# PhyloStar/CyBayes

Measured on NVIDIA B200. Metric: tree log-likelihood evals/sec, higher is better.
Workload: dtype f64

## Files before the change

### cybayes_b200/csrc/cybayes_b200.cu

```cuda
#include <cuda_runtime.h>
#include <dlfcn.h>
#include <limits.h>
#include <stdarg.h>
#include <stdio.h>
#include <stdlib.h>
#include <string.h>

#include <time.h>

#include <algorithm>
#include <exception>
#include <new>
#include <string>
#include <vector>

#include "cb_types.cuh"
#include "kernels_dmma.cuh"
#include "kernels_dmma_rc.cuh"
#include "kernels_general.cuh"
#include "kernels_pmat.cuh"
#include "kernels_s2.cuh"
#include "kernels_s2t.cuh"

using namespace cb;
// ... 36 lines not shown
  } catch (...) {
    return fail("internal error: unknown exception");
  }
}

struct NcclId { char internal[128]; };
typedef struct ncclComm* ncclComm_t;
struct NcclApi {
  void* lib = nullptr;
  int (*GetUniqueId)(NcclId*) = nullptr;
  int (*CommInitRank)(ncclComm_t*, int, NcclId, int) = nullptr;
  int (*AllReduce)(const void*, void*, size_t, int, int, ncclComm_t, cudaStream_t) = nullptr;
  int (*AllGather)(const void*, void*, size_t, int, ncclComm_t, cudaStream_t) = nullptr;
  int (*CommDestroy)(ncclComm_t) = nullptr;
  const char* (*GetErrorString)(int) = nullptr;
};
static NcclApi g_nccl;
static int load_nccl() {
  if (g_nccl.lib) return 0;
  const char* names[] = {"libnccl.so.2", "libnccl.so"};
  for (const char* n : names) {
    g_nccl.lib = dlopen(n, RTLD_NOW | RTLD_GLOBAL);
    if (g_nccl.lib) break;
  }
  REQUIRE(g_nccl.lib, "cannot dlopen libnccl.so.2: %s", dlerror());
  g_nccl.GetUniqueId = (int (*)(NcclId*))dlsym(g_nccl.lib, "ncclGetUniqueId");
  g_nccl.CommInitRank = (int (*)(ncclComm_t*, int, NcclId, int))dlsym(g_nccl.lib, "ncclCommInitRank");
  g_nccl.AllReduce = (int (*)(const void*, void*, size_t, int, int, ncclComm_t, cudaStream_t))dlsym(g_nccl.lib, "ncclAllReduce");
  g_nccl.AllGather = (int (*)(const void*, void*, size_t, int, ncclComm_t, cudaStream_t))dlsym(g_nccl.lib, "ncclAllGather");
  g_nccl.CommDestroy = (int (*)(ncclComm_t))dlsym(g_nccl.lib, "ncclCommDestroy");
  g_nccl.GetErrorString = (const char* (*)(int))dlsym(g_nccl.lib, "ncclGetErrorString");
  REQUIRE(g_nccl.GetUniqueId && g_nccl.CommInitRank && g_nccl.AllReduce && g_nccl.CommDestroy,
          "libnccl is missing expected symbols");
  return 0;
}
enum { NCCL_DOUBLE = 8, NCCL_SUM = 0, NCCL_INT8 = 0 };

constexpr int DMMA_RC_MIN_STATES = 9;
constexpr int64_t DMMA_RC_MIN_SITES = 1024;
constexpr int64_t S2_TILED_MIN_SITES = 64 * 2 * 148 * 4;

struct Buffer {
  double* data = nullptr;
  int32_t* scale = nullptr;
  int refs = 0;
};
struct Snapshot {
  std::vector<int32_t> buf_of_node;
  std::vector<int32_t> cherry_of_node;
  int refs = 0;
};
struct CherryRec {
  int32_t tip[2] = {0, 0};
  int refs = 0;
};

struct PlanChild {
  int32_t kind;
  int32_t ref;
  int32_t edge;
};
struct PlanOp {
  int32_t node;
  PlanChild ch[2];
  int32_t out_buf;
  int32_t pf_buf;
  uint8_t is_root, keep, stream, spill, pushed;
  uint8_t make_rec;
  uint8_t synthetic;
};
struct PlanLaunch { int r_begin, r_end, max_ops, n_bufs; };
struct EvalPlan {
  int flags = 0, n_lists = 0, split_env = 0;
  std::vector<int32_t> key_offsets, key_nodes, key_children;
  std::vector<PlanOp> ops;
  std::vector<RangeDesc> ranges;
  std::vector<PlanLaunch> launches;
  int64_t bytes_written = 0, bytes_read = 0;
  int n_stored = 0, n_buffer_reads = 0, n_stack = 0, n_spills = 0, n_cherries = 0, n_small_recs = 0;
  uint64_t stamp = 0;
};
constexpr int PLAN_FLAG_MASK = CB_EVAL_WANT_SNAPSHOT | CB_EVAL_STORE_ROOT | CB_EVAL_FORCE_LEVELS | CB_EVAL_FORCE_WALK | CB_EVAL_NO_FOLD;
constexpr int PLAN_CACHE_SIZE = 6;

struct cb_ctx {
  int device = 0;
  cudaStream_t stream = nullptr;
  cudaEvent_t ev0 = nullptr, ev1 = nullptr, ev_stage = nullptr, ev_mark[2] = {nullptr, nullptr};
  int sm_count = 148;
  int n_taxa = 0, n_states = 0, n_cats = 0, code_bytes = 1, n_amb = 0;
  int64_t n_sites = 0, P = 0;
  bool family_s2 = false;
  bool use_dmma = false;
  bool dmma_rc = false;
  int rc_stagger = 1;
  double* d_staged = nullptr;
  size_t staged_bytes = 0;
  bool s2_tiled = false;
  int s2t_slots = 3;
  int s2t_minb = 3;
  int s2t_v = 2;
  bool s2t_bulk = false;
  bool s2t_prefetch = true;
  bool s2t_small_recs = true;
  S2TImage* d_images = nullptr;
  int s2_vec = 1;
  int s2_minb = 3;
  bool s2_stream_stores = true;
  void* d_codes = nullptr;
  double* d_weights = nullptr;
  double* d_amb = nullptr;
  double* d_pi = nullptr;
  double* d_pmats = nullptr;
  int pmat_cap = 0;
  std::vector<Buffer> buffers;
  std::vector<int> free_buffers;
  size_t buffer_bytes = 0;
  std::vector<Snapshot> snaps;
  std::vector<int> free_snaps;
  std::vector<CherryRec> recs;
  std::vector<int> free_recs;
  double* d_pmats_lib = nullptr;
  int lib_cap = 0;
  unsigned char* h_stage = nullptr;
  unsigned char* d_stage = nullptr;
  size_t stage_cap = 0;
  int images_cap = 0;
  cudaEvent_t ev_scratch = nullptr;
  bool timing = true;
  bool results_mapped = false;
  double* d_block_sums = nullptr;
  unsigned* d_tickets = nullptr;
  double* d_results = nullptr;
  double* h_results = nullptr;
  double* d_root_dot = nullptr;
  int32_t* d_root_exp = nullptr;
  int out_cap = 0, max_blocks = 0;
  int last_n_out = 0;
  void* d_scratch = nullptr;
  void* h_scratch = nullptr;
  size_t scratch_cap = 0;
  void* d_flush = nullptr;
  size_t flush_bytes = 0;
  ncclComm_t comm = nullptr;
  int n_ranks = 1, rank = 0;
  bool fused_allreduce = false;
  Mail* d_mailbox = nullptr;
  Mail** d_peer_mailbox = nullptr;
  std::vector<void*> peer_opened;
  int32_t* d_comm_error = nullptr;
  unsigned long long epoch = 0;
  std::vector<EvalPlan> plans;
  EvalPlan scratch_plan;
  uint64_t plan_clock = 0, plan_builds = 0;
  bool no_plan_cache = false;
  std::vector<int> work_new_bufs, work_new_nodes, work_cherry_nodes;
  cudaEvent_t ev_main0 = nullptr, ev_main1 = nullptr;
// ... 23 lines not shown
  dev_account(c->device, (int64_t)bytes);
  return 0;
}
static void dev_free(cb_ctx* c, void* p, size_t bytes) {
  if (p) {
    cudaFree(p);
    c->dev_bytes -= (int64_t)bytes;
    dev_account(c->device, -(int64_t)bytes);
  }
}

extern "C" const char* cb_last_error(void) { return g_err.c_str(); }
extern "C" int cb_version(void) { return 100; }
extern "C" int cb_device_count(int* out) {
  REQUIRE(out, "null argument");
  CU(cudaGetDeviceCount(out));
  return 0;
}

static int create_impl(int device, cb_ctx** out);
extern "C" int cb_create(int device, cb_ctx** out) {
  return guarded([&] { return create_impl(device, out); });
}
static int create_impl(int device, cb_ctx** out) {
  REQUIRE(out, "null argument");
  int n = 0;
  cudaError_t e = cudaGetDeviceCount(&n);
  if (e != cudaSuccess || n == 0)
    return fail("no CUDA device available (%s); cybayes_b200 has no CPU fallback", cudaGetErrorString(e));
  REQUIRE(device >= 0 && device < n, "device %d out of range (have %d)", device, n);
  CU(cudaSetDevice(device));
  cb_ctx* c = new cb_ctx();
  c->device = device;
  CU(cudaStreamCreateWithFlags(&c->stream, cudaStreamNonBlocking));
  CU(cudaEventCreate(&c->ev0));
  CU(cudaEventCreate(&c->ev1));
  CU(cudaEventCreateWithFlags(&c->ev_stage, cudaEventDisableTiming));
  CU(cudaEventCreate(&c->ev_mark[0]));
  CU(cudaEventCreate(&c->ev_mark[1]));
  CU(cudaEventCreateWithFlags(&c->ev_scratch, cudaEventDisableTiming));
  CU(cudaEventCreate(&c->ev_main0));
  CU(cudaEventCreate(&c->ev_main1));
  cudaDeviceProp prop;
  CU(cudaGetDeviceProperties(&prop, device));
  c->sm_count = prop.multiProcessorCount;
  if (const char* v = getenv("CYBAYES_S2_V")) c->s2_vec = (atoi(v) == 2) ? 2 : 1;
  if (const char* v = getenv("CYBAYES_S2_MINB")) c->s2_minb = (atoi(v) == 4) ? 4 : 3;
  if (getenv("CYBAYES_S2_NO_CS")) c->s2_stream_stores = false;
  if (const char* v = getenv("CYBAYES_S2T_MINB")) c->s2t_minb = std::max(2, std::min(4, atoi(v)));
  if (const char* v = getenv("CYBAYES_S2T_V")) c->s2t_v = atoi(v) == 2 ? 2 : 1;
  if (c->s2t_minb == 4) c->s2t_v = 1;
  if (getenv("CYBAYES_S2T_BULK")) c->s2t_bulk = atoi(getenv("CYBAYES_S2T_BULK")) != 0;
  if (getenv("CYBAYES_S2T_PREFETCH")) c->s2t_prefetch = atoi(getenv("CYBAYES_S2T_PREFETCH")) != 0;
  if (getenv("CYBAYES_S2T_SMALL_RECS")) c->s2t_small_recs = atoi(getenv("CYBAYES_S2T_SMALL_RECS")) != 0;
  c->s2t_slots = c->s2t_minb == 4 ? 2 : c->s2t_minb == 3 ? 3 : 4;
  if (const char* v = getenv("CYBAYES_S2T_SLOTS")) c->s2t_slots = std::max(0, std::min(8, atoi(v)));
  if (getenv("CYBAYES_NO_PLAN_CACHE")) c->no_plan_cache = true;
  if (const char* v = getenv("CYBAYES_MAX_DEVICE_BYTES")) c->max_dev_bytes = atoll(v);
#define CB_S2T_ATTR(CC, MB, VV) CU(cudaFuncSetAttribute(prune_s2t_kernel<CC, MB, VV>, cudaFuncAttributeMaxDynamicSharedMemorySize, 226 * 1024))
  CB_S2T_ATTR(4, 2, 1); CB_S2T_ATTR(4, 3, 1); CB_S2T_ATTR(1, 2, 1); CB_S2T_ATTR(1, 3, 1);
  CB_S2T_ATTR(4, 2, 2); CB_S2T_ATTR(1, 2, 2); CB_S2T_ATTR(4, 3, 2); CB_S2T_ATTR(1, 3, 2); CB_S2T_ATTR(4, 4, 1); CB_S2T_ATTR(1, 4, 1);
#undef CB_S2T_ATTR
  CU(cudaFuncSetAttribute(prune_general_kernel, cudaFuncAttributeMaxDynamicSharedMemorySize, 227 * 1024));
#define CB_DMMA_ATTR(SS) CU(cudaFuncSetAttribute(prune_dmma_kernel<SS>, cudaFuncAttributeMaxDynamicSharedMemorySize, 227 * 1024))
  CB_DMMA_ATTR(0); CB_DMMA_ATTR(32); CB_DMMA_ATTR(40); CB_DMMA_ATTR(47); CB_DMMA_ATTR(48); CB_DMMA_ATTR(56); CB_DMMA_ATTR(64);
#undef CB_DMMA_ATTR
#define CB_RC_ATTR(SS)                                                                                                          \
  CU(cudaFuncSetAttribute(prune_dmma_rc_kernel<SS, true>, cudaFuncAttributeMaxDynamicSharedMemorySize, (int)RcCfg<SS>::SMEM)); \
  CU(cudaFuncSetAttribute(prune_dmma_rc_kernel<SS, false>, cudaFuncAttributeMaxDynamicSharedMemorySize, (int)RcCfg<SS>::SMEM))
  CB_RC_ATTR(16); CB_RC_ATTR(24); CB_RC_ATTR(32); CB_RC_ATTR(40); CB_RC_ATTR(48); CB_RC_ATTR(56); CB_RC_ATTR(64);
#undef CB_RC_ATTR
  if (const char* v = getenv("CYBAYES_RC_STAGGER")) c->rc_stagger = atoi(v) != 0;
  *out = c;
  return 0;
}

static void free_alignment(cb_ctx* c) {
  c->plans.clear();
  if (c->d_images) dev_free(c, c->d_images, (size_t)c->images_cap * sizeof(S2TImage));
  c->d_images = nullptr;
  c->images_cap = 0;
  for (auto& b : c->buffers) dev_free(c, b.data, c->buffer_bytes);
  c->buffers.clear();
  c->free_buffers.clear();
  c->snaps.clear();
  c->free_snaps.clear();
  c->recs.clear();
  c->free_recs.clear();
  if (c->d_pmats_lib) dev_free(c, c->d_pmats_lib, (size_t)c->lib_cap * 2 * c->n_cats * c->n_states * c->n_states * 8);
  c->d_pmats_lib = nullptr;
  c->lib_cap = 0;
  if (c->d_codes) dev_free(c, c->d_codes, (size_t)c->n_taxa * c->P * c->code_bytes);
  if (c->d_weights) dev_free(c, c->d_weights, (size_t)c->P * 8);
  if (c->d_amb) dev_free(c, c->d_amb, (size_t)std::max(1, c->n_amb) * c->n_states * 8);
  if (c->d_pi) dev_free(c, c->d_pi, (size_t)c->n_states * 8);
  if (c->d_pmats) dev_free(c, c->d_pmats, (size_t)c->pmat_cap * c->n_states * c->n_states * 8);
  if (c->d_staged) dev_free(c, c->d_staged, c->staged_bytes);
  c->d_staged = nullptr;
  c->staged_bytes = 0;
  c->d_codes = nullptr;
  c->d_weights = c->d_amb = c->d_pi = c->d_pmats = nullptr;
  c->pmat_cap = 0;
  if (c->d_block_sums) dev_free(c, c->d_block_sums, (size_t)c->out_cap * c->max_blocks * 8);
  if (c->d_tickets) dev_free(c, c->d_tickets, (size_t)c->out_cap * 4);
  if (c->d_results) dev_free(c, c->d_results, (size_t)c->out_cap * 8);
  if (c->d_root_dot) dev_free(c, c->d_root_dot, (size_t)c->out_cap * c->n_cats * c->P * 8);
  if (c->d_root_exp) dev_free(c, c->d_root_exp, (size_t)c->out_cap * c->n_cats * c->P * 4);
// ... 243 lines not shown
  if (check_slots(c, count, slots)) return 1;
  REQUIRE(d, "null argument");
  REQUIRE(model >= CB_MODEL_JC && model <= CB_MODEL_GTR_EIG, "unknown model %d", model);
  REQUIRE(model == CB_MODEL_JC || pi, "pi required");
  REQUIRE(model != CB_MODEL_GTR_EIG || gtr, "GTR eigensystem required");
  REQUIRE(model != CB_MODEL_F81_BINARY || c->n_states == 2, "binary F81 needs 2 states");
  if (count == 0) return 0;
  CU(cudaSetDevice(c->device));
  const int S = c->n_states;
  const size_t n_gtr = (model == CB_MODEL_GTR_EIG) ? (size_t)S + 2 * (size_t)S * S : 0;
  const size_t doubles = (size_t)S + n_gtr + 2 * (size_t)count;
  const size_t bytes = doubles * 8 + (size_t)count * 4;
  if (ensure_scratch(c, bytes)) return 1;
  CU(cudaEventSynchronize(c->ev_scratch));
  double* h = (double*)c->h_scratch;
  if (pi) memcpy(h, pi, (size_t)S * 8); else memset(h, 0, (size_t)S * 8);
  if (n_gtr) memcpy(h + S, gtr, n_gtr * 8);
  memcpy(h + S + n_gtr, d, (size_t)count * 8);
  if (x) memcpy(h + S + n_gtr + count, x, (size_t)count * 8);
  memcpy(h + doubles, slots, (size_t)count * 4);
  CU(cudaMemcpyAsync(c->d_scratch, c->h_scratch, bytes, cudaMemcpyHostToDevice, c->stream));
  CU(cudaEventRecord(c->ev_scratch, c->stream));
  c->h2d += (int64_t)bytes;
  const double* dd = (const double*)c->d_scratch;
  const int threads = (S * S >= 256) ? 256 : ((S * S + 31) / 32 * 32);
  pmat_build_kernel<<<count, threads, (size_t)S * 8, c->stream>>>(
      model, S, dd, beta, n_gtr ? dd + S : nullptr, count, (const int32_t*)(dd + doubles), dd + S + n_gtr,
      x ? dd + S + n_gtr + count : nullptr, c->d_pmats);
  CU(cudaGetLastError());
  c->launches += 1;
  return 0;
}

static int buffer_acquire(cb_ctx* c, int* out) {
  if (!c->free_buffers.empty()) {
    *out = c->free_buffers.back();
    c->free_buffers.pop_back();
  } else {
    Buffer b;
    void* p = nullptr;
    if (dev_alloc(c, &p, c->buffer_bytes)) return 1;
    b.data = (double*)p;
    b.scale = (int32_t*)(b.data + (size_t)c->n_cats * c->n_states * c->P);
    c->buffers.push_back(b);
    *out = (int)c->buffers.size() - 1;
  }
  c->buffers[*out].refs = 1;
  return 0;
}
static void buffer_release(cb_ctx* c, int b) {
  if (b < 0) return;
  if (--c->buffers[b].refs == 0) c->free_buffers.push_back(b);
}
static int rec_acquire(cb_ctx* c, int tip0, int tip1, int* out) {
  if (!c->free_recs.empty()) {
    *out = c->free_recs.back();
    c->free_recs.pop_back();
  } else {
    c->recs.emplace_back();
    *out = (int)c->recs.size() - 1;
  }
  c->recs[*out].tip[0] = tip0;
  c->recs[*out].tip[1] = tip1;
  c->recs[*out].refs = 1;
  return 0;
}
static void rec_release(cb_ctx* c, int r) {
  if (r < 0) return;
  if (--c->recs[r].refs == 0) c->free_recs.push_back(r);
}
static int ensure_lib_pool(cb_ctx* c) {
  const int need = (int)c->recs.size();
  if (need <= c->lib_cap) return 0;
  const int cap = std::max(need, std::max(1024, c->lib_cap * 2));
  const size_t per = (size_t)2 * c->n_cats * c->n_states * c->n_states * 8;
  double* nd = nullptr;
  if (dev_alloc(c, (void**)&nd, (size_t)cap * per)) return 1;
  if (c->d_pmats_lib) {
    CU(cudaMemcpyAsync(nd, c->d_pmats_lib, (size_t)c->lib_cap * per, cudaMemcpyDeviceToDevice, c->stream));
    CU(cudaStreamSynchronize(c->stream));
    dev_free(c, c->d_pmats_lib, (size_t)c->lib_cap * per);
  }
  c->d_pmats_lib = nd;
  c->lib_cap = cap;
  return 0;
}
static bool snapshot_valid(cb_ctx* c, int s) {
  return s >= 0 && s < (int)c->snaps.size() && c->snaps[s].refs > 0;
}
extern "C" int cb_snapshot_retain(cb_ctx* c, int s) {
  REQUIRE(c && snapshot_valid(c, s), "invalid snapshot %d", s);
  c->snaps[s].refs++;
  return 0;
}
extern "C" int cb_snapshot_release(cb_ctx* c, int s) {
  REQUIRE(c && snapshot_valid(c, s), "invalid snapshot %d", s);
  if (--c->snaps[s].refs == 0) {
    for (int32_t b : c->snaps[s].buf_of_node) buffer_release(c, b);
    for (int32_t r : c->snaps[s].cherry_of_node) rec_release(c, r);
    c->snaps[s].buf_of_node.clear();
    c->snaps[s].cherry_of_node.clear();
    c->free_snaps.push_back(s);
  }
  return 0;
}

static int snapshot_read_impl(cb_ctx* c, int s, int node, double* out, int32_t* scale_out);
extern "C" int cb_snapshot_read(cb_ctx* c, int s, int node, double* out, int32_t* scale_out) {
  return guarded([&] { return snapshot_read_impl(c, s, node, out, scale_out); });
}
static int materialize_cherry(cb_ctx* c, const Snapshot& sn, int rec, int* buf_out);
static int snapshot_read_impl(cb_ctx* c, int s, int node, double* out, int32_t* scale_out) {
  REQUIRE(c && out && snapshot_valid(c, s), "invalid snapshot %d", s);
  const Snapshot& sn = c->snaps[s];
  REQUIRE(node >= 0 && node < (int)sn.buf_of_node.size(), "node %d is not in snapshot %d", node, s);
  CU(cudaSetDevice(c->device));
// ... 177 lines not shown
#define CB_LAUNCH_S2(CC, VV, TT, MB) prune_s2_kernel<CC, VV, TT, MB><<<grid, TT, smem, c->stream>>>(kk)
    if (c->n_cats == 4) {
      if (small) CB_LAUNCH_S2(4, 1, 64, 8);
      else if (V == 1 && c->s2_minb == 4) CB_LAUNCH_S2(4, 1, 256, 4);
      else if (V == 1) CB_LAUNCH_S2(4, 1, 256, 3);
      else CB_LAUNCH_S2(4, 2, 256, 2);
    } else {
      if (small) CB_LAUNCH_S2(1, 1, 64, 8); else if (V == 1) CB_LAUNCH_S2(1, 1, 256, 4); else CB_LAUNCH_S2(1, 2, 256, 4);
    }
#undef CB_LAUNCH_S2
  } else if (c->dmma_rc) {
    dim3 grid((unsigned)((c->P + RC_T - 1) / RC_T), (unsigned)n_r, (unsigned)c->n_cats);
    switch ((c->n_states + 7) / 8 * 8) {
#define CB_RC_CASE(SS)                                                                                          \
  case SS:                                                                                                      \
    if (c->n_states == SS) prune_dmma_rc_kernel<SS, true><<<grid, RC_THREADS, RcCfg<SS>::SMEM, c->stream>>>(kk); \
    else prune_dmma_rc_kernel<SS, false><<<grid, RC_THREADS, RcCfg<SS>::SMEM, c->stream>>>(kk);                  \
    break
      CB_RC_CASE(16); CB_RC_CASE(24); CB_RC_CASE(32); CB_RC_CASE(40); CB_RC_CASE(48); CB_RC_CASE(56); CB_RC_CASE(64);
#undef CB_RC_CASE
      default: return fail("internal error: no register-carried DMMA kernel for %d states", c->n_states);
    }
  } else if (c->use_dmma) {
    dim3 grid((unsigned)(c->P / DM_T), (unsigned)n_r, (unsigned)c->n_cats);
    const size_t smem = dm_smem_bytes(c->n_states);
    switch (c->n_states) {
#define CB_DMMA_CASE(SS) case SS: prune_dmma_kernel<SS><<<grid, DM_THREADS, smem, c->stream>>>(kk); break
      CB_DMMA_CASE(32); CB_DMMA_CASE(40); CB_DMMA_CASE(47); CB_DMMA_CASE(48); CB_DMMA_CASE(56); CB_DMMA_CASE(64);
#undef CB_DMMA_CASE
      default: prune_dmma_kernel<0><<<grid, DM_THREADS, smem, c->stream>>>(kk);
    }
  } else {
    const int R = general_rows_per_chunk(c->n_states);
    REQUIRE(R > 0, "n_states = %d does not fit the shared-memory tiling", c->n_states);
    dim3 grid((unsigned)(c->P / GEN_T), (unsigned)n_r, (unsigned)c->n_cats);
    prune_general_kernel<<<grid, GEN_THREADS, gen_smem_bytes(c->n_states, R), c->stream>>>(kk, R);
  }
  CU(cudaGetLastError());
  c->launches += 1;
  return 0;
}

static int launch_images(cb_ctx* c, const LaunchConst& k, int n_ops) {
  if (!c->s2_tiled) return 0;
  if (c->n_cats == 4) s2t_image_kernel<4><<<n_ops, 32, 0, c->stream>>>(k, n_ops, c->d_images);
  else s2t_image_kernel<1><<<n_ops, 32, 0, c->stream>>>(k, n_ops, c->d_images);
  CU(cudaGetLastError());
  c->launches += 1;
  return 0;
}

static int materialize_cherry(cb_ctx* c, const Snapshot& sn, int rec, int* buf_out) {
  REQUIRE(c->family_s2 && rec >= 0 && rec < (int)c->recs.size(), "bad record %d", rec);
  if (ensure_staging(c, 1, 1, 1)) return 1;
  CU(cudaStreamSynchronize(c->stream));
  int bi;
  if (buffer_acquire(c, &bi)) return 1;
  OpDesc& op = *reinterpret_cast<OpDesc*>(c->h_stage);
  memset(&op, 0, sizeof op);
  op.dst = c->buffers[bi].data;
  op.dst_scale = c->buffers[bi].scale;
  op.out_buf = op.pf_buf = op.frec_out = -1;
  const int C = c->n_cats, N = c->n_taxa;
  const size_t row_bytes = (size_t)c->P * c->code_bytes;
  int order[2] = {0, 1};
  if (c->s2_tiled && c->recs[rec].tip[0] > N && c->recs[rec].tip[1] <= N) { order[0] = 1; order[1] = 0; }
  for (int w = 0; w < 2; ++w) {
    const int kx = order[w], ch = c->recs[rec].tip[kx];
    for (int q = 0; q < C; ++q) op.pslot[w][q] = CB_LIB_SLOT | (rec * 2 * C + kx * C + q);
    op.crec_out[w] = -1;
    if (ch <= N) {
      op.kind[w] = SRC_TIP;
      op.src[w] = (const char*)c->d_codes + (size_t)(ch - 1) * row_bytes;
    } else {
      const int yrec = ch < (int)sn.cherry_of_node.size() ? sn.cherry_of_node[ch] : -1;
      if (yrec < 0) { buffer_release(c, bi); return fail("internal error: cherry %d of record %d is not in the snapshot", ch, rec); }
      op.kind[w] = SRC_CHERRY;
      for (int t = 0; t < 2; ++t) {
        op.ctip[w][t] = (const char*)c->d_codes + (size_t)(c->recs[yrec].tip[t] - 1) * row_bytes;
        for (int q = 0; q < CB_S2_MAX_CATS; ++q) op.cslot[w][t][q] = q < C ? (CB_LIB_SLOT | (yrec * 2 * C + t * C + q)) : 0;
      }
    }
  }
  *reinterpret_cast<RangeDesc*>(c->h_stage + sizeof(OpDesc)) = RangeDesc{0, 1, -1, 0};
  CU(cudaMemcpyAsync(c->d_stage, c->h_stage, sizeof(OpDesc) + sizeof(RangeDesc), cudaMemcpyHostToDevice, c->stream));
  LaunchConst k = make_const(c);
  k.ranges = reinterpret_cast<const RangeDesc*>(c->d_stage + sizeof(OpDesc));
  if (launch_images(c, k, 1)) { buffer_release(c, bi); return 1; }
  if (launch_ranges(c, k, 0, 1, 1, 0)) { buffer_release(c, bi); return 1; }
  CU(cudaStreamSynchronize(c->stream));
  *buf_out = bi;
  return 0;
}

enum Schedule { SCHED_CHAIN = 0, SCHED_WALK = 1, SCHED_LEVELS = 2 };


static int build_plan(cb_ctx* c, const Snapshot* sin, int n_lists, const int32_t* offsets_in, const int32_t* nodes_in,
                      const int32_t* children_in, int flags, EvalPlan& plan) {
  const int N = c->n_taxa, n_nodes = 2 * N;
  const bool fold = c->family_s2 && !(flags & CB_EVAL_NO_FOLD);
  const bool want_snap = (flags & CB_EVAL_WANT_SNAPSHOT) != 0;
  const bool store_root = (flags & CB_EVAL_STORE_ROOT) != 0;
  const int C = c->n_cats;
  const int K = c->s2_tiled ? c->s2t_slots : 0;
  const int slot_base = c->s2t_bulk ? S2T_STAGING : 0;
  plan.ops.clear(); plan.ranges.clear(); plan.launches.clear();
  plan.bytes_written = plan.bytes_read = 0;
  plan.n_stored = plan.n_buffer_reads = plan.n_stack = plan.n_spills = plan.n_cherries = plan.n_small_recs = 0;
  const int64_t tip_row_bytes = c->P * c->code_bytes;

  struct LOp { int32_t node, caller; int32_t child[2], folded[2]; };
  std::vector<LOp> L;
  std::vector<int32_t> parent_op(n_nodes), folded_at(n_nodes), op_of_node(n_nodes, -1);
  std::vector<int> kid[2], n_sub, order, pos_of, range_id, push_slot, first_kid, level_of, by_level;
  std::vector<std::pair<int, int>> segs;
  std::vector<int> seg_of;
  std::vector<int> f;
  std::vector<char> read_back;
  bool single_launch = true;

  for (int li = 0; li < n_lists; ++li) {
    const int b_in = offsets_in[li], e_in = offsets_in[li + 1];
    REQUIRE(e_in > b_in, "empty op list %d", li);
    L.clear();
    std::fill(parent_op.begin(), parent_op.end(), -1);
    std::fill(folded_at.begin(), folded_at.end(), -1);
    for (int i = b_in; i < e_in; ++i)
      for (int kx = 0; kx < 2; ++kx) {
        const int ch = children_in[2 * i + kx];
        REQUIRE((ch >= 1 && ch <= N) || (ch > N && ch < n_nodes), "op %d: bad child id %d", i, ch);
        if (ch > N) parent_op[ch] = i;
      }
    for (int i = b_in; i < e_in; ++i) {
      const int node = nodes_in[i], c0 = children_in[2 * i], c1 = children_in[2 * i + 1];
      REQUIRE(node > N && node < n_nodes, "op %d: node %d is not an internal node", i, node);
      const bool cherry = fold && c0 <= N && c1 <= N && i != e_in - 1 && parent_op[node] > i;
      if (cherry) {
        folded_at[node] = i;
        plan.n_cherries++;
        continue;
      }
      LOp o;
      o.node = node;
      o.caller = i;
      for (int kx = 0; kx < 2; ++kx) {
        const int ch = children_in[2 * i + kx];
        o.child[kx] = ch;
        o.folded[kx] = ch > N ? folded_at[ch] : -1;
      }
      L.push_back(o);
    }
    if (sin && c->s2_tiled) {
      std::vector<LOp> syn;
      auto is_rec = [&](int nd) { return nd > N && nd < (int)sin->cherry_of_node.size() && sin->cherry_of_node[nd] >= 0; };
      for (const LOp& o : L)
        for (int kx = 0; kx < 2; ++kx) {
          const int ch = o.child[kx];
          if (ch <= N || o.folded[kx] >= 0 || !is_rec(ch)) continue;
          const CherryRec& r = c->recs[sin->cherry_of_node[ch]];
          if (r.tip[0] <= N && r.tip[1] <= N) continue;
          bool in_list = false;
          for (const LOp& q : L) in_list = in_list || q.node == ch;
          if (in_list) continue;
          LOp so;
          so.node = ch;
          so.caller = ~sin->cherry_of_node[ch];
          so.child[0] = r.tip[0]; so.child[1] = r.tip[1];
          so.folded[0] = so.folded[1] = -1;
          syn.push_back(so);
        }
      if (!syn.empty()) L.insert(L.begin(), syn.begin(), syn.end());
    }
    const int n = (int)L.size();
    for (int j = 0; j < n; ++j) {
      REQUIRE(op_of_node[L[j].node] < 0, "op %d: node %d is computed twice", L[j].caller, L[j].node);
      op_of_node[L[j].node] = j;
    }
    auto cleanup = [&] { for (int j = 0; j < n; ++j) op_of_node[L[j].node] = -1; };
    kid[0].assign(n, -1);
    kid[1].assign(n, -1);
    for (int j = 0; j < n; ++j)
      for (int kx = 0; kx < 2; ++kx) {
        const int ch = L[j].child[kx];
        if (ch > N && L[j].folded[kx] < 0 && op_of_node[ch] >= 0) {
          if (op_of_node[ch] >= j) { cleanup(); return fail("op %d: child %d is computed after its parent", L[j].caller, ch); }
          kid[kx][j] = op_of_node[ch];
        } else if (ch > N && L[j].folded[kx] < 0) {
          const bool in_snap = sin && ch < (int)sin->buf_of_node.size() &&
                               (sin->buf_of_node[ch] >= 0 || (ch < (int)sin->cherry_of_node.size() && sin->cherry_of_node[ch] >= 0));
          if (!in_snap) { cleanup(); return fail("op %d: child %d is neither recomputed nor in the input snapshot", L[j].caller, ch); }
        }
      }
    cleanup();
    bool chain = !(flags & CB_EVAL_FORCE_LEVELS) && n <= MAX_CHAIN_OPS;
    for (int j = 0; j < n && chain; ++j) {
      const int a0 = kid[0][j], a1 = kid[1][j];
      if (j == 0) chain = (a0 < 0 && a1 < 0);
      else chain = (a0 == j - 1) != (a1 == j - 1) && (a0 < 0 || a0 == j - 1) && (a1 < 0 || a1 == j - 1);
    }
    Schedule sched = SCHED_CHAIN;
    if (!chain) {
      const bool big = c->dmma_rc || c->P >= (c->family_s2 ? WALK_MIN_SITES_S2 : WALK_MIN_SITES_GENERAL);
      sched = ((big || n_lists > 1 || (flags & CB_EVAL_FORCE_WALK)) && !(flags & CB_EVAL_FORCE_LEVELS)) ? SCHED_WALK : SCHED_LEVELS;
      if (n_lists > 1 && sched == SCHED_LEVELS) return fail("cb_eval_batch: candidate %d is not a chain (level schedule forced)", li);
    }

    order.resize(n);
    for (int j = 0; j < n; ++j) order[j] = j;
    seg_of.assign(n, 0);
    push_slot.assign(n, -1);
    segs.clear();
    if (sched == SCHED_WALK) {
      n_sub.assign(n, 1);
      for (int j = 0; j < n; ++j)
        for (int kx = 0; kx < 2; ++kx)
          if (kid[kx][j] >= 0) n_sub[j] += n_sub[kid[kx][j]];
      bool rooted = (n_sub[n - 1] == n);
      if (!rooted) {
        REQUIRE(n_lists == 1, "cb_eval_batch: candidate %d has ops that are not under its root", li);
        sched = SCHED_LEVELS;
      } else {
        int limit = n + 1;
        if (n_lists == 1) {
// ... 11 lines not shown
        std::vector<int> cut, top, stack;
        if (limit <= n) {
          stack.push_back(n - 1);
          while (!stack.empty()) {
            const int j = stack.back();
            stack.pop_back();
            if (n_sub[j] <= limit) { cut.push_back(j); continue; }
            for (int kx = 0; kx < 2; ++kx)
              if (kid[kx][j] >= 0) stack.push_back(kid[kx][j]);
          }
          std::stable_sort(cut.begin(), cut.end(), [&](int x, int y) { return n_sub[x] > n_sub[y]; });
          for (size_t s = 0; s < cut.size(); ++s) {
            stack.push_back(cut[s]);
            while (!stack.empty()) {
              const int j = stack.back();
              stack.pop_back();
              seg_of[j] = (int)s + 1;
              for (int kx = 0; kx < 2; ++kx)
                if (kid[kx][j] >= 0) stack.push_back(kid[kx][j]);
            }
          }
        }
        f.assign((size_t)n * (K + 1), 0);
        first_kid.assign((size_t)n * (K + 1), 0);
        for (int j = 0; j < n; ++j) {
          int a = kid[0][j], b2 = kid[1][j];
          if (a >= 0 && seg_of[a] != seg_of[j]) a = -1;
          if (b2 >= 0 && seg_of[b2] != seg_of[j]) b2 = -1;
          for (int kk = 0; kk <= K; ++kk) {
            int& fj = f[(size_t)j * (K + 1) + kk];
            if (a >= 0 && b2 >= 0) {
              const int k1 = kk > 0 ? kk - 1 : 0, miss = kk == 0 ? 1 : 0;
              const int ca = f[(size_t)a * (K + 1) + kk] + miss + f[(size_t)b2 * (K + 1) + k1];
              const int cb2 = f[(size_t)b2 * (K + 1) + kk] + miss + f[(size_t)a * (K + 1) + k1];
              const bool a_first = ca < cb2 || (ca == cb2 && n_sub[a] >= n_sub[b2]);
              fj = a_first ? ca : cb2;
              first_kid[(size_t)j * (K + 1) + kk] = a_first ? 0 : 1;
              const int cs = f[(size_t)a * (K + 1) + kk] + 1 + f[(size_t)b2 * (K + 1) + kk];
              if (kk > 0 && cs < fj) {
                fj = cs;
                first_kid[(size_t)j * (K + 1) + kk] = (n_sub[a] >= n_sub[b2] ? 0 : 1) | 2;
              }
            } else if (a >= 0) {
              fj = f[(size_t)a * (K + 1) + kk];
            } else if (b2 >= 0) {
              fj = f[(size_t)b2 * (K + 1) + kk];
            }
          }
        }
        std::vector<int> out;
        out.reserve(n);
        struct Frame { int j, k, phase; };
        std::vector<Frame> fr;
        auto emit = [&](int root_op) {
          fr.push_back({root_op, K, 0});
          while (!fr.empty()) {
            Frame& t = fr.back();
            const int j = t.j, kk = t.k;
            int a = kid[0][j], b2 = kid[1][j];
            if (a >= 0 && seg_of[a] != seg_of[j]) a = -1;
            if (b2 >= 0 && seg_of[b2] != seg_of[j]) b2 = -1;
            if (a >= 0 && b2 >= 0) {
              const int fk = first_kid[(size_t)j * (K + 1) + kk];
              const bool push = kk > 0 && !(fk & 2);
              const int x = (fk & 1) == 0 ? a : b2, y = (fk & 1) == 0 ? b2 : a;
              if (t.phase == 0) { t.phase = 1; fr.push_back({x, kk, 0}); continue; }
              if (t.phase == 1) {
                push_slot[x] = push ? slot_base + (K - kk) : -1;
                t.phase = 2;
                fr.push_back({y, push ? kk - 1 : kk, 0});
                continue;
              }
            } else if (a >= 0 || b2 >= 0) {
              if (t.phase == 0) { t.phase = 2; fr.push_back({a >= 0 ? a : b2, kk, 0}); continue; }
            }
            out.push_back(j);
            fr.pop_back();
          }
        };
        if (limit > n) {
          emit(n - 1);
        } else {
          for (int r : cut) {
            const int b0 = (int)out.size();
            emit(r);
            segs.push_back({b0, (int)out.size()});
          }
          emit(n - 1);
        }
        REQUIRE((int)out.size() == n, "internal error: walk order covers %d of %d ops", (int)out.size(), n);
        order = out;
      }
    }
    pos_of.assign(n, 0);
    for (int p = 0; p < n; ++p) pos_of[order[p]] = p;
    range_id.assign(n, 0);
    for (size_t si = 0; si < segs.size(); ++si)
      for (int p = segs[si].first; p < segs[si].second; ++p) range_id[p] = (int)si + 1;
    auto same_range = [&](int p0, int p1) { return sched != SCHED_LEVELS && range_id[p0] == range_id[p1]; };

    read_back.assign(n, 0);
    const int base = (int)plan.ops.size();
    plan.ops.resize(base + n);
    int staging_rr = 0;
    for (int p = 0; p < n; ++p) {
      const int j = order[p];
      PlanOp& po = plan.ops[base + p];
      po.node = L[j].node;
      po.is_root = (j == n - 1);
      REQUIRE(!po.is_root || p == n - 1, "internal error: root is not last");
      po.keep = po.stream = po.spill = po.pushed = po.make_rec = 0;
      po.synthetic = L[j].caller < 0 ? 1 : 0;
      po.out_buf = po.pf_buf = -1;
      for (int kx = 0; kx < 2; ++kx) {
        PlanChild& pc = po.ch[kx];
        const int ch = L[j].child[kx];
        pc.edge = L[j].caller >= 0 ? 2 * L[j].caller + kx : ~((~L[j].caller) * 2 * C + kx * C);
        if (ch <= N) {
          pc.kind = SRC_TIP;
          pc.ref = ch;
          plan.bytes_read += tip_row_bytes;
        } else if (L[j].folded[kx] >= 0) {
          pc.kind = SRC_CHERRY;
          pc.ref = L[j].folded[kx];
          plan.bytes_read += 2 * tip_row_bytes;
        } else if (kid[kx][j] >= 0) {
          const int jj = kid[kx][j], pp = pos_of[jj];
          if (same_range(pp, p) && pp == p - 1) {
            pc.kind = SRC_CARRIED;
            pc.ref = 0;
          } else if (same_range(pp, p) && push_slot[jj] >= 0) {
            pc.kind = SRC_STACK;
            pc.ref = push_slot[jj];
            plan.n_stack++;
          } else {
            REQUIRE(pp < p, "internal error: producer of node %d runs after its consumer", ch);
            pc.kind = SRC_BUFFER;
            pc.ref = base + pp;
            read_back[jj] = same_range(pp, p) ? 2 : 1;
            plan.bytes_read += (int64_t)c->buffer_bytes;
            plan.n_buffer_reads++;
          }
        } else {
          const bool rec = fold && sin && ch < (int)sin->cherry_of_node.size() && sin->cherry_of_node[ch] >= 0;
          pc.kind = rec ? SRC_CHERRY : SRC_BUFFER;
          pc.ref = ~ch;
          plan.bytes_read += rec ? 2 * tip_row_bytes : (int64_t)c->buffer_bytes;
          if (!rec) plan.n_buffer_reads++;
        }
      }
    }
    plan.bytes_read += c->P * 8;
    if (c->s2_tiled)
      for (int p = 0; p < n; ++p) {
        PlanOp& po = plan.ops[base + p];
        if (s2t_rank(po.ch[1].kind) < s2t_rank(po.ch[0].kind)) std::swap(po.ch[0], po.ch[1]);
        REQUIRE(s2t_combo(po.ch[0].kind, po.ch[1].kind) >= 0, "internal error: op of node %d has children of kinds %d, %d", po.node,
                po.ch[0].kind, po.ch[1].kind);
      }
    for (int p = 0; p < n; ++p) {
      const int j = order[p];
      PlanOp& po = plan.ops[base + p];
      po.keep = po.is_root ? (want_snap && store_root) : ((want_snap && !po.synthetic) || read_back[j] != 0);
      po.stream = (po.keep && read_back[j] == 0 && c->s2_stream_stores) ? 1 : 0;
      po.spill = (read_back[j] == 2) ? 1 : 0;
      if (po.keep) {
        plan.bytes_written += (int64_t)c->buffer_bytes;
        plan.n_stored++;
        if (po.spill) plan.n_spills++;
      }
      if (c->s2_tiled && c->s2t_small_recs && want_snap && po.keep && !po.is_root && !po.synthetic && read_back[j] == 0 &&
          (po.ch[0].kind == SRC_TIP || po.ch[0].kind == SRC_CHERRY) && po.ch[1].kind == SRC_CHERRY) {
        po.keep = 0;
        po.stream = 0;
        po.make_rec = 1;
        plan.bytes_written -= (int64_t)c->buffer_bytes;
        plan.n_stored--;
        plan.n_small_recs++;
      }
      if (c->s2_tiled) {
        if (push_slot[j] >= 0 && !po.is_root) { po.out_buf = push_slot[j]; po.pushed = 1; }
        else if (c->s2t_bulk && po.keep && !po.spill) { po.out_buf = staging_rr; staging_rr ^= 1; }
      }
    }
    int max_slot = -1;
    for (int j = 0; j < n; ++j) max_slot = std::max(max_slot, push_slot[j]);
    if (c->s2_tiled && c->s2t_prefetch && max_slot < 2 && !c->s2t_bulk) {
      const int pf_base = max_slot + 1;
      int rr = 0;
      for (int p = 0; p < n; ++p) {
        PlanOp& po = plan.ops[base + p];
        if (po.ch[0].kind != SRC_CARRIED || po.ch[1].kind != SRC_BUFFER) continue;
        const int ref = po.ch[1].ref;
        const bool other_launch = ref < 0 || !same_range(ref - base, p);
        if (!other_launch) continue;
        po.ch[1].kind = SRC_STACK;
        po.pf_buf = pf_base + rr;
        rr = (rr + 1) % 3;
      }
    }

    auto bufs_of = [&](int p0, int p1) {
      int nb = 0;
      for (int p = p0; p < p1; ++p) {
        const PlanOp& po = plan.ops[base + p];
        nb = std::max(nb, std::max(po.out_buf, po.pf_buf) + 1);
        for (int kx = 0; kx < 2; ++kx)
          if (po.ch[kx].kind == SRC_STACK && po.pf_buf < 0) nb = std::max(nb, po.ch[kx].ref + 1);
      }
      return nb;
    };
    if (sched == SCHED_WALK && !segs.empty()) {
      single_launch = false;
      const int start = (int)plan.ranges.size();
      int mx = 1, nb = 0;
      for (auto& sg : segs) {
        plan.ranges.push_back(RangeDesc{base + sg.first, base + sg.second, -1, 0});
        mx = std::max(mx, sg.second - sg.first);
        nb = std::max(nb, bufs_of(sg.first, sg.second));
      }
      plan.launches.push_back({start, (int)plan.ranges.size(), mx, nb});
      const int tb = segs.back().second;
      plan.ranges.push_back(RangeDesc{base + tb, base + n, li, 0});
      plan.launches.push_back({(int)plan.ranges.size() - 1, (int)plan.ranges.size(), n - tb, bufs_of(tb, n)});
    } else if (sched != SCHED_LEVELS) {
      plan.ranges.push_back(RangeDesc{base, base + n, li, 0});
    } else {
      single_launch = false;
// ... 138 lines not shown
      if (want_snap) {
        new_bufs.push_back(bi);
        new_nodes.push_back(po.node);
      }
    }
    for (int kx = 0; kx < 2; ++kx) {
      const PlanChild& pc = po.ch[kx];
      op.kind[kx] = pc.kind;
      op.src[kx] = nullptr;
      op.src_scale[kx] = nullptr;
      op.ctip[kx][0] = op.ctip[kx][1] = nullptr;
      op.crec_out[kx] = -1;
      op.in_buf[kx] = -1;
      if (pc.edge >= 0) {
        const int32_t* ps = pslots_in + (size_t)pc.edge * C;
        for (int q = 0; q < C; ++q) op.pslot[kx][q] = ps[q];
      } else {
        for (int q = 0; q < C; ++q) op.pslot[kx][q] = CB_LIB_SLOT | (~pc.edge + q);
      }
      for (int q = C; q < CB_MAX_CATS; ++q) op.pslot[kx][q] = 0;
      switch (pc.kind) {
        case SRC_TIP:
          op.src[kx] = codes + (size_t)(pc.ref - 1) * row_bytes;
          break;
        case SRC_BUFFER:
          if (pc.ref >= 0) {
            op.src[kx] = h_ops[pc.ref].dst;
            op.src_scale[kx] = h_ops[pc.ref].dst_scale;
          } else {
            const Buffer& bf = c->buffers[sin->buf_of_node[~pc.ref]];
            op.src[kx] = bf.data;
            op.src_scale[kx] = bf.scale;
          }
          break;
        case SRC_STACK:
          if (po.pf_buf >= 0 && kx == 1) {
            op.in_buf[kx] = po.pf_buf;
            op.src[kx] = pc.ref >= 0 ? (const void*)h_ops[pc.ref].dst : (const void*)c->buffers[sin->buf_of_node[~pc.ref]].data;
          } else {
            op.in_buf[kx] = pc.ref;
          }
          break;
        case SRC_CHERRY:
          if (pc.ref >= 0) {
            const int fo = pc.ref;
            for (int t = 0; t < 2; ++t) {
              const int tip = children_in[2 * fo + t];
              op.ctip[kx][t] = codes + (size_t)(tip - 1) * row_bytes;
              const int32_t* cs = pslots_in + (size_t)(2 * fo + t) * C;
              for (int q = 0; q < CB_S2_MAX_CATS; ++q) op.cslot[kx][t][q] = q < C ? cs[q] : 0;
            }
            if (want_snap) {
              int r;
              if (rec_acquire(c, children_in[2 * fo], children_in[2 * fo + 1], &r)) return 1;
              guard.recs.push_back(r);
              op.crec_out[kx] = r;
              new_cherry_nodes.push_back(nodes_in[fo]);
            }
          } else {
            const int rec = sin->cherry_of_node[~pc.ref];
            for (int t = 0; t < 2; ++t) {
              op.ctip[kx][t] = codes + (size_t)(c->recs[rec].tip[t] - 1) * row_bytes;
              for (int q = 0; q < CB_S2_MAX_CATS; ++q) op.cslot[kx][t][q] = q < C ? (CB_LIB_SLOT | (rec * 2 * C + t * C + q)) : 0;
            }
          }
          break;
        default: break;
      }
    }
    if (po.make_rec) {
      int ids[2];
      for (int kx = 0; kx < 2; ++kx) {
        const PlanChild& pc = po.ch[kx];
        ids[kx] = pc.kind == SRC_TIP ? pc.ref : (pc.ref >= 0 ? nodes_in[pc.ref] : ~pc.ref);
      }
      int r;
      if (rec_acquire(c, ids[0], ids[1], &r)) return 1;
      guard.recs.push_back(r);
      op.frec_out = r;
      new_cherry_nodes.push_back(po.node);
    }
  }
  memcpy(c->h_stage + off_ranges, plan->ranges.data(), (size_t)n_ranges * sizeof(RangeDesc));
  memcpy(c->h_stage + off_pi, pi, (size_t)c->n_states * 8);

  const double t_filled = now_us();
  if (ensure_lib_pool(c)) return 1;
  const size_t stage_bytes = off_pi + (size_t)c->n_states * 8;
  CU(cudaMemcpyAsync(c->d_stage, c->h_stage, stage_bytes, cudaMemcpyHostToDevice, c->stream));
  CU(cudaEventRecord(c->ev_stage, c->stream));
  c->h2d += (int64_t)stage_bytes;

  if (c->dmma_rc) {
    const int S8 = (c->n_states + 7) / 8 * 8;
    const size_t need = (size_t)total_ops * 2 * C * (S8 + RC_EXTRA_ROWS) * S8 * 8;
    if (need > c->staged_bytes) {
      CU(cudaStreamSynchronize(c->stream));
      if (c->d_staged) dev_free(c, c->d_staged, c->staged_bytes);
      c->d_staged = nullptr;
      c->staged_bytes = 0;
      const size_t cap = std::max(need, (size_t)64 << 20);
      if (dev_alloc(c, (void**)&c->d_staged, cap)) return 1;
      c->staged_bytes = cap;
    }
  }
  LaunchConst k = make_const(c);
  k.ranges = reinterpret_cast<const RangeDesc*>(c->d_stage + off_ranges);
  k.pi = reinterpret_cast<const double*>(c->d_stage + off_pi);
  const bool fused = c->comm != nullptr && c->fused_allreduce && n_lists <= CB_MB_OUTS;
  if (fused) {
    k.n_ranks = c->n_ranks;
    k.my_rank = c->rank;
    k.epoch = ++c->epoch;
    k.mailbox = c->d_mailbox;
    k.peer_mailbox = c->d_peer_mailbox;
    k.comm_error = c->d_comm_error;
  }
  const bool mapped = c->comm == nullptr || fused;
  if (mapped) {
    double* dev_view = nullptr;
    CU(cudaHostGetDevicePointer((void**)&dev_view, c->h_results, 0));
    k.results = dev_view;
  }
  if (c->timing) CU(cudaEventRecord(c->ev0, c->stream));
  if (c->dmma_rc) {
    const unsigned jobs = (unsigned)(total_ops * 2 * C);
    switch ((c->n_states + 7) / 8 * 8) {
#define CB_RS_CASE(SS) case SS: rc_restage_kernel<SS><<<jobs, 256, 0, c->stream>>>(k, total_ops, c->d_staged); break
      CB_RS_CASE(16); CB_RS_CASE(24); CB_RS_CASE(32); CB_RS_CASE(40); CB_RS_CASE(48); CB_RS_CASE(56); CB_RS_CASE(64);
#undef CB_RS_CASE
// ... 472 lines not shown
```

Baseline: 163.2.

## Generalize small-record recomputation to deeper subtrees with cost-bounded selection

Extends the 'small record' mechanism, which skips storing partial-likelihood buffers for snapshot nodes and recomputes them from tip codes later. Records can now cover nested subtrees whose recomputation cost, times sibling tip count, stays under a threshold (default 8). Synthetic recompute ops are expanded recursively, and materialization recurses through nested records. It also adjusts the push-slot starting depth when prefetch is on. Fewer buffer writes cut memory traffic, in exchange for extra recomputation and more synthetic ops.

```diff
diff --git a/cybayes_b200/csrc/cybayes_b200.cu b/cybayes_b200/csrc/cybayes_b200.cu
--- a/cybayes_b200/csrc/cybayes_b200.cu
+++ b/cybayes_b200/csrc/cybayes_b200.cu
@@ -112,6 +112,7 @@
 };
 struct CherryRec {
   int32_t tip[2] = {0, 0};
+  int32_t cost = 0;
   int refs = 0;
 };
 
@@ -119,6 +120,7 @@
   int32_t kind;
   int32_t ref;
   int32_t edge;
+  int32_t node;
 };
 struct PlanOp {
   int32_t node;
@@ -128,6 +130,7 @@
   uint8_t is_root, keep, stream, spill, pushed;
   uint8_t make_rec;
   uint8_t synthetic;
+  int32_t cost;
 };
 struct PlanLaunch { int r_begin, r_end, max_ops, n_bufs; };
 struct EvalPlan {
@@ -162,7 +165,7 @@
   int s2t_v = 2;
   bool s2t_bulk = false;
   bool s2t_prefetch = true;
-  bool s2t_small_recs = true;
+  int s2t_small_recs = 8;
   S2TImage* d_images = nullptr;
   int s2_vec = 1;
   int s2_minb = 3;
@@ -292,7 +295,7 @@
   if (c->s2t_minb == 4) c->s2t_v = 1;
   if (getenv("CYBAYES_S2T_BULK")) c->s2t_bulk = atoi(getenv("CYBAYES_S2T_BULK")) != 0;
   if (getenv("CYBAYES_S2T_PREFETCH")) c->s2t_prefetch = atoi(getenv("CYBAYES_S2T_PREFETCH")) != 0;
-  if (getenv("CYBAYES_S2T_SMALL_RECS")) c->s2t_small_recs = atoi(getenv("CYBAYES_S2T_SMALL_RECS")) != 0;
+  if (getenv("CYBAYES_S2T_SMALL_RECS")) c->s2t_small_recs = std::max(0, atoi(getenv("CYBAYES_S2T_SMALL_RECS")));
   c->s2t_slots = c->s2t_minb == 4 ? 2 : c->s2t_minb == 3 ? 3 : 4;
   if (const char* v = getenv("CYBAYES_S2T_SLOTS")) c->s2t_slots = std::max(0, std::min(8, atoi(v)));
   if (getenv("CYBAYES_NO_PLAN_CACHE")) c->no_plan_cache = true;
@@ -642,7 +645,7 @@
   if (b < 0) return;
   if (--c->buffers[b].refs == 0) c->free_buffers.push_back(b);
 }
-static int rec_acquire(cb_ctx* c, int tip0, int tip1, int* out) {
+static int rec_acquire(cb_ctx* c, int tip0, int tip1, int cost, int* out) {
   if (!c->free_recs.empty()) {
     *out = c->free_recs.back();
     c->free_recs.pop_back();
@@ -652,6 +655,7 @@
   }
   c->recs[*out].tip[0] = tip0;
   c->recs[*out].tip[1] = tip1;
+  c->recs[*out].cost = cost;
   c->recs[*out].refs = 1;
   return 0;
 }
@@ -935,33 +939,45 @@
 
 static int materialize_cherry(cb_ctx* c, const Snapshot& sn, int rec, int* buf_out) {
   REQUIRE(c->family_s2 && rec >= 0 && rec < (int)c->recs.size(), "bad record %d", rec);
-  if (ensure_staging(c, 1, 1, 1)) return 1;
+  const int C = c->n_cats, N = c->n_taxa;
+  int yrec[2] = {-1, -1}, tmp[2] = {-1, -1};
+  auto release_tmp = [&] { buffer_release(c, tmp[0]); buffer_release(c, tmp[1]); };
+  for (int kx = 0; kx < 2; ++kx) {
+    const int ch = c->recs[rec].tip[kx];
+    if (ch <= N) continue;
+    yrec[kx] = ch < (int)sn.cherry_of_node.size() ? sn.cherry_of_node[ch] : -1;
+    if (yrec[kx] < 0) { release_tmp(); return fail("internal error: child %d of record %d is not in the snapshot", ch, rec); }
+    const CherryRec& y = c->recs[yrec[kx]];
+    if ((y.tip[0] > N || y.tip[1] > N) && materialize_cherry(c, sn, yrec[kx], &tmp[kx])) { release_tmp(); return 1; }
+  }
+  if (ensure_staging(c, 1, 1, 1)) { release_tmp(); return 1; }
   CU(cudaStreamSynchronize(c->stream));
   int bi;
-  if (buffer_acquire(c, &bi)) return 1;
+  if (buffer_acquire(c, &bi)) { release_tmp(); return 1; }
   OpDesc& op = *reinterpret_cast<OpDesc*>(c->h_stage);
   memset(&op, 0, sizeof op);
   op.dst = c->buffers[bi].data;
   op.dst_scale = c->buffers[bi].scale;
   op.out_buf = op.pf_buf = op.frec_out = -1;
-  const int C = c->n_cats, N = c->n_taxa;
   const size_t row_bytes = (size_t)c->P * c->code_bytes;
+  auto kind_of = [&](int kx) { return c->recs[rec].tip[kx] <= N ? SRC_TIP : tmp[kx] >= 0 ? SRC_BUFFER : SRC_CHERRY; };
   int order[2] = {0, 1};
-  if (c->s2_tiled && c->recs[rec].tip[0] > N && c->recs[rec].tip[1] <= N) { order[0] = 1; order[1] = 0; }
+  if (c->s2_tiled && s2t_rank(kind_of(1)) < s2t_rank(kind_of(0))) { order[0] = 1; order[1] = 0; }
   for (int w = 0; w < 2; ++w) {
     const int kx = order[w], ch = c->recs[rec].tip[kx];
     for (int q = 0; q < C; ++q) op.pslot[w][q] = CB_LIB_SLOT | (rec * 2 * C + kx * C + q);
     op.crec_out[w] = -1;
-    if (ch <= N) {
-      op.kind[w] = SRC_TIP;
+    op.in_buf[w] = -1;
+    op.kind[w] = kind_of(kx);
+    if (op.kind[w] == SRC_TIP) {
       op.src[w] = (const char*)c->d_codes + (size_t)(ch - 1) * row_bytes;
+    } else if (op.kind[w] == SRC_BUFFER) {
+      op.src[w] = c->buffers[tmp[kx]].data;
+      op.src_scale[w] = c->buffers[tmp[kx]].scale;
     } else {
-      const int yrec = ch < (int)sn.cherry_of_node.size() ? sn.cherry_of_node[ch] : -1;
-      if (yrec < 0) { buffer_release(c, bi); return fail("internal error: cherry %d of record %d is not in the snapshot", ch, rec); }
-      op.kind[w] = SRC_CHERRY;
       for (int t = 0; t < 2; ++t) {
-        op.ctip[w][t] = (const char*)c->d_codes + (size_t)(c->recs[yrec].tip[t] - 1) * row_bytes;
-        for (int q = 0; q < CB_S2_MAX_CATS; ++q) op.cslot[w][t][q] = q < C ? (CB_LIB_SLOT | (yrec * 2 * C + t * C + q)) : 0;
+        op.ctip[w][t] = (const char*)c->d_codes + (size_t)(c->recs[yrec[kx]].tip[t] - 1) * row_bytes;
+        for (int q = 0; q < CB_S2_MAX_CATS; ++q) op.cslot[w][t][q] = q < C ? (CB_LIB_SLOT | (yrec[kx] * 2 * C + t * C + q)) : 0;
       }
     }
   }
@@ -969,9 +985,9 @@
   CU(cudaMemcpyAsync(c->d_stage, c->h_stage, sizeof(OpDesc) + sizeof(RangeDesc), cudaMemcpyHostToDevice, c->stream));
   LaunchConst k = make_const(c);
   k.ranges = reinterpret_cast<const RangeDesc*>(c->d_stage + sizeof(OpDesc));
-  if (launch_images(c, k, 1)) { buffer_release(c, bi); return 1; }
-  if (launch_ranges(c, k, 0, 1, 1, 0)) { buffer_release(c, bi); return 1; }
+  if (launch_images(c, k, 1) || launch_ranges(c, k, 0, 1, 1, 0)) { buffer_release(c, bi); release_tmp(); return 1; }
   CU(cudaStreamSynchronize(c->stream));
+  release_tmp();
   *buf_out = bi;
   return 0;
 }
@@ -996,6 +1012,8 @@
   struct LOp { int32_t node, caller; int32_t child[2], folded[2]; };
   std::vector<LOp> L;
   std::vector<int32_t> parent_op(n_nodes), folded_at(n_nodes), op_of_node(n_nodes, -1);
+  std::vector<char> in_list(n_nodes, 0), is_rec;
+  std::vector<int> cost, tips, sib_tips;
   std::vector<int> kid[2], n_sub, order, pos_of, range_id, push_slot, first_kid, level_of, by_level;
   std::vector<std::pair<int, int>> segs;
   std::vector<int> seg_of;
@@ -1036,23 +1054,27 @@
     }
     if (sin && c->s2_tiled) {
       std::vector<LOp> syn;
-      auto is_rec = [&](int nd) { return nd > N && nd < (int)sin->cherry_of_node.size() && sin->cherry_of_node[nd] >= 0; };
+      for (const LOp& o : L) in_list[o.node] = 1;
+      auto needs_op = [&](int nd) {
+        if (nd <= N || in_list[nd] || nd >= (int)sin->cherry_of_node.size() || sin->cherry_of_node[nd] < 0) return false;
+        const CherryRec& r = c->recs[sin->cherry_of_node[nd]];
+        return r.tip[0] > N || r.tip[1] > N;
+      };
+      auto expand = [&](auto&& self, int nd) -> void {
+        const CherryRec& r = c->recs[sin->cherry_of_node[nd]];
+        for (int kx = 0; kx < 2; ++kx)
+          if (needs_op(r.tip[kx])) self(self, r.tip[kx]);
+        LOp so;
+        so.node = nd;
+        so.caller = ~sin->cherry_of_node[nd];
+        so.child[0] = r.tip[0]; so.child[1] = r.tip[1];
+        so.folded[0] = so.folded[1] = -1;
+        syn.push_back(so);
+      };
       for (const LOp& o : L)
-        for (int kx = 0; kx < 2; ++kx) {
-          const int ch = o.child[kx];
-          if (ch <= N || o.folded[kx] >= 0 || !is_rec(ch)) continue;
-          const CherryRec& r = c->recs[sin->cherry_of_node[ch]];
-          if (r.tip[0] <= N && r.tip[1] <= N) continue;
-          bool in_list = false;
-          for (const LOp& q : L) in_list = in_list || q.node == ch;
-          if (in_list) continue;
-          LOp so;
-          so.node = ch;
-          so.caller = ~sin->cherry_of_node[ch];
-          so.child[0] = r.tip[0]; so.child[1] = r.tip[1];
-          so.folded[0] = so.folded[1] = -1;
-          syn.push_back(so);
-        }
+        for (int kx = 0; kx < 2; ++kx)
+          if (o.folded[kx] < 0 && needs_op(o.child[kx])) expand(expand, o.child[kx]);
+      for (const LOp& o : L) in_list[o.node] = 0;
       if (!syn.empty()) L.insert(L.begin(), syn.begin(), syn.end());
     }
     const int n = (int)L.size();
@@ -1170,8 +1192,10 @@
         out.reserve(n);
         struct Frame { int j, k, phase; };
         std::vector<Frame> fr;
+        int k0 = K;
+        if (sin && limit > n && c->s2t_prefetch && K > 2 && f[(size_t)(n - 1) * (K + 1) + 2] == f[(size_t)(n - 1) * (K + 1) + K]) k0 = 2;
         auto emit = [&](int root_op) {
-          fr.push_back({root_op, K, 0});
+          fr.push_back({root_op, k0, 0});
           while (!fr.empty()) {
             Frame& t = fr.back();
             const int j = t.j, kk = t.k;
@@ -1184,7 +1208,7 @@
               const int x = (fk & 1) == 0 ? a : b2, y = (fk & 1) == 0 ? b2 : a;
               if (t.phase == 0) { t.phase = 1; fr.push_back({x, kk, 0}); continue; }
               if (t.phase == 1) {
-                push_slot[x] = push ? slot_base + (K - kk) : -1;
+                push_slot[x] = push ? slot_base + (k0 - kk) : -1;
                 t.phase = 2;
                 fr.push_back({y, push ? kk - 1 : kk, 0});
                 continue;
@@ -1233,6 +1257,7 @@
       for (int kx = 0; kx < 2; ++kx) {
         PlanChild& pc = po.ch[kx];
         const int ch = L[j].child[kx];
+        pc.node = ch;
         pc.edge = L[j].caller >= 0 ? 2 * L[j].caller + kx : ~((~L[j].caller) * 2 * C + kx * C);
         if (ch <= N) {
           pc.kind = SRC_TIP;
@@ -1276,22 +1301,54 @@
         REQUIRE(s2t_combo(po.ch[0].kind, po.ch[1].kind) >= 0, "internal error: op of node %d has children of kinds %d, %d", po.node,
                 po.ch[0].kind, po.ch[1].kind);
       }
+    cost.assign(n, 0);
+    is_rec.assign(n, 0);
+    constexpr int NOT_SMALL = 1 << 20;
+    tips.assign(n, 0);
+    sib_tips.assign(n, NOT_SMALL);
+    auto child_tips = [&](int j, int kx) -> int {
+      const int ch = L[j].child[kx];
+      if (ch <= N) return 1;
+      if (L[j].folded[kx] >= 0) return 2;
+      if (kid[kx][j] >= 0) return tips[kid[kx][j]];
+      const bool cherry = sin && ch < (int)sin->cherry_of_node.size() && sin->cherry_of_node[ch] >= 0;
+      return cherry ? 2 : NOT_SMALL;
+    };
+    for (int j = 0; j < n; ++j) {
+      tips[j] = std::min(NOT_SMALL, child_tips(j, 0) + child_tips(j, 1));
+      for (int kx = 0; kx < 2; ++kx)
+        if (kid[kx][j] >= 0) sib_tips[kid[kx][j]] = child_tips(j, 1 - kx);
+    }
     for (int p = 0; p < n; ++p) {
       const int j = order[p];
       PlanOp& po = plan.ops[base + p];
       po.keep = po.is_root ? (want_snap && store_root) : ((want_snap && !po.synthetic) || read_back[j] != 0);
       po.stream = (po.keep && read_back[j] == 0 && c->s2_stream_stores) ? 1 : 0;
       po.spill = (read_back[j] == 2) ? 1 : 0;
+      po.cost = 0;
       if (po.keep) {
         plan.bytes_written += (int64_t)c->buffer_bytes;
         plan.n_stored++;
         if (po.spill) plan.n_spills++;
       }
-      if (c->s2_tiled && c->s2t_small_recs && want_snap && po.keep && !po.is_root && !po.synthetic && read_back[j] == 0 &&
-          (po.ch[0].kind == SRC_TIP || po.ch[0].kind == SRC_CHERRY) && po.ch[1].kind == SRC_CHERRY) {
+      cost[j] = 1;
+      for (int kx = 0; kx < 2; ++kx) {
+        const int ch = L[j].child[kx];
+        if (ch <= N || L[j].folded[kx] >= 0) continue;
+        if (kid[kx][j] >= 0) cost[j] += is_rec[kid[kx][j]] ? cost[kid[kx][j]] : NOT_SMALL;
+        else if (!(sin && ch < (int)sin->cherry_of_node.size() && sin->cherry_of_node[ch] >= 0)) cost[j] += NOT_SMALL;
+      }
+      if (po.synthetic) cost[j] = c->recs[~L[j].caller].cost;
+      is_rec[j] = po.synthetic && !po.keep;
+      const int R = c->s2t_small_recs;
+      const bool small = R > 0 && (cost[j] <= 1 || (int64_t)cost[j] * sib_tips[j] <= R);
+      if (c->s2_tiled && fold && want_snap && po.keep && !po.is_root && !po.synthetic && read_back[j] == 0 && small &&
+          !(L[j].child[0] <= N && L[j].child[1] <= N)) {
         po.keep = 0;
         po.stream = 0;
         po.make_rec = 1;
+        po.cost = cost[j];
+        is_rec[j] = 1;
         plan.bytes_written -= (int64_t)c->buffer_bytes;
         plan.n_stored--;
         plan.n_small_recs++;
@@ -1536,7 +1593,7 @@
             }
             if (want_snap) {
               int r;
-              if (rec_acquire(c, children_in[2 * fo], children_in[2 * fo + 1], &r)) return 1;
+              if (rec_acquire(c, children_in[2 * fo], children_in[2 * fo + 1], 0, &r)) return 1;
               guard.recs.push_back(r);
               op.crec_out[kx] = r;
               new_cherry_nodes.push_back(nodes_in[fo]);
@@ -1553,13 +1610,8 @@
       }
     }
     if (po.make_rec) {
-      int ids[2];
-      for (int kx = 0; kx < 2; ++kx) {
-        const PlanChild& pc = po.ch[kx];
-        ids[kx] = pc.kind == SRC_TIP ? pc.ref : (pc.ref >= 0 ? nodes_in[pc.ref] : ~pc.ref);
-      }
       int r;
-      if (rec_acquire(c, ids[0], ids[1], &r)) return 1;
+      if (rec_acquire(c, po.ch[0].node, po.ch[1].node, po.cost, &r)) return 1;
       guard.recs.push_back(r);
       op.frec_out = r;
       new_cherry_nodes.push_back(po.node);
```

Result: faster. 179.3, median of 6 (+9.9%).
